# ankitkumar93/compute-war

Measured on AMD Instinct MI355X. Metric: GB/s ingested (Skein-512 + LZ4, 64 KiB blocks), higher is better.
Workload: dtype u64; 1 GPU; skein512+lz4, 1048576 x 65536 B uniform-random blocks/GPU in HBM; blocks_per_gpu=1048576, block_bytes=65536, parallelism=block-sharded x1, gather-only RCCL

## Files before the change

### compute_war_amd/csrc/lz4_kernel.hip

```cpp

#include <hip/hip_runtime.h>
#include <stdint.h>
#include <stdio.h>
#include <stdlib.h>
#include <string.h>

#include <type_traits>

#include "cw_device.h"
#include "lz_device.h"
#include "stream_scratch.h"

#ifndef HEADW_GLOBAL
#define HEADW_GLOBAL 16
#endif
#ifndef HEADW_STAGED
#define HEADW_STAGED 64
#endif

namespace cw {

using lz::Around;
using lz::around;
using lz::copy_g2g;
// ... 193 lines not shown
        const uint32_t off = c * kChunk + j * 1024 + lane * 16;
        if (c < nchunks && off < n) r.p[j] = *reinterpret_cast<const uint4 *>(g + off);
    }
}
__device__ __forceinline__ void chunk_stage(const Chunk &r, uint32_t *ring32, uint32_t c, uint32_t n, uint32_t lane)
{
#pragma unroll
    for (uint32_t j = 0; j < kPieces; j++) {
        const uint32_t off = c * kChunk + j * 1024 + lane * 16;
        if (off < n) *reinterpret_cast<uint4 *>(reinterpret_cast<uint8_t *>(ring32) + (off & (kRing - 1))) = r.p[j];
    }
}
__device__ __forceinline__ void chunk_store(const Chunk &r, uint8_t *lit, uint32_t c, uint32_t n, uint32_t lane)
{
#pragma unroll
    for (uint32_t j = 0; j < kPieces; j++) {
        const uint32_t off = c * kChunk + j * 1024 + lane * 16;
        if (off < n) {
            uint32_t *q = reinterpret_cast<uint32_t *>(lit + off);
            __builtin_nontemporal_store(r.p[j].x, q);
            __builtin_nontemporal_store(r.p[j].y, q + 1);
            __builtin_nontemporal_store(r.p[j].z, q + 2);
            __builtin_nontemporal_store(r.p[j].w, q + 3);
        }
    }
}

struct Walk {
    ScanState st;
    uint32_t knext = 0, v0 = 0;
    bool marked = false;
};

template <int NG>
__device__ __forceinline__ void probe_groups(Walk &w, const uint32_t (&pos)[kStreamGroup], const bool (&act)[kStreamGroup], uint32_t *tab,
                                             const uint32_t *ring32, uint32_t tag, uint32_t epoch)
{
    uint32_t v[NG], old[NG];
#pragma unroll
    for (int j = 0; j < NG; j++) {
        const uint32_t a0 = (pos[j] & (kRing - 1)) >> 2, a1 = (a0 + 1) & (kRing / 4 - 1);
        v[j] = __builtin_amdgcn_alignbyte(ring32[a1], ring32[a0], pos[j] & 3u);
    }
#pragma unroll
    for (int j = 0; j < NG; j++) old[j] = scan_issue(tab, tag, pos[j], v[j], act[j]);
#pragma unroll
    for (int j = 0; j < NG; j++) scan_judge(old[j], epoch, w.v0, pos[j], v[j], act[j], w.st);
}

__device__ __forceinline__ void probe_upto(Walk &w, uint32_t end, uint32_t *tab, const uint32_t *ring32, uint32_t tag, uint32_t epoch,
                                           uint32_t nprobes, const uint8_t *g, uint32_t lane)
{
    for (;;) {
        uint32_t pos[kStreamGroup], nact = 0, ngroups = 0;
        bool act[kStreamGroup];
#pragma unroll
        for (uint32_t j = 0; j < kStreamGroup; j++) {
            const uint32_t k = w.knext + 64 * j + lane;
            pos[j] = 1 + probe_delta(k);
            act[j] = k < nprobes && pos[j] < end;
            const unsigned long long m = __ballot(act[j]);
            nact += (uint32_t)__builtin_popcountll(m);
            ngroups += m != 0;
        }
        if (nact == 0) return;
        if (ngroups == 1) probe_groups<1>(w, pos, act, tab, ring32, tag, epoch);
        else if (ngroups == 2) probe_groups<2>(w, pos, act, tab, ring32, tag, epoch);
        else probe_groups<kStreamGroup>(w, pos, act, tab, ring32, tag, epoch);
        w.marked = scan_settle(g, w.st);
        w.knext += nact;
        if (w.marked || nact < 64 * kStreamGroup) return;
    }
}

__global__ void __launch_bounds__(64)
lz4_scan_stream_kernel(const uint8_t *__restrict__ src, uint32_t n, size_t src_stride, size_t nblocks,
                       uint8_t *__restrict__ dst, size_t dst_stride, uint32_t *__restrict__ sizes, uint32_t nprobes,
                       uint32_t *__restrict__ queue, uint32_t *__restrict__ counters, size_t first_block, uint32_t feed_word)
{
    __shared__ __attribute__((aligned(16))) uint32_t tab[1u << 13];
    __shared__ __attribute__((aligned(16))) uint32_t ring32[kRing / 4];
    volatile uint32_t *mailbox = ring32;
    const uint32_t lane = threadIdx.x;
    __builtin_amdgcn_s_setprio(3);
    uint32_t epoch = 15;
    const uint32_t nchunks = (n + kChunk - 1) / kChunk;
    const uint32_t hdr = 1 + (n >= 15 ? (n - 15) / 255 + 1 : 0);

    BlockFeed feed;
    const uint32_t run = n >= 65536 ? 1u : 65536u / n;
    for (size_t rel; scan_next_block(feed, rel, counters + feed_word - 2, mailbox, run, nblocks - first_block, lane);) {
        const size_t blk = first_block + rel;
        scan_begin_block(tab, epoch, lane);
        const uint8_t *g = src + blk * src_stride;
        uint8_t *out = dst + blk * dst_stride, *lit = out + hdr;
        const uint32_t tag = epoch << 28;
        Walk w;
        Chunk r0, r1, r2;

#define CW_STAGE(PREV, CUR, C)                                                                         \
        do {                                                                                           \
            const uint32_t c_ = (C);                                                                   \
            if (c_) chunk_store(PREV, lit, c_ - 1, n, lane);                                           \
            chunk_load(PREV, g, c_ + 2, nchunks, n, lane);                                             \
            chunk_stage(CUR, ring32, c_, n, lane);                                                     \
            if (c_ == 0) {                                                                             \
                w.v0 = ring32[0];                                                                      \
                if (nprobes && lane == 0) {                                                            \
                    const uint32_t h0 = w.v0 * 2654435761u;                                            \
                    atomicMax(&tab[h0 >> 19], tag | ((h0 >> 7) & 0xFFFu));             \
                }                                                                                      \
            } else {                                                                                   \
                probe_upto(w, c_ * kChunk, tab, ring32, tag, epoch, nprobes, g, lane);                 \
            }                                                                                          \
        } while (0)

        chunk_load(r0, g, 0, nchunks, n, lane);
        chunk_load(r1, g, 1, nchunks, n, lane);
        for (uint32_t c = 0; c < nchunks && !w.marked; c += 3) {
            CW_STAGE(r2, r0, c);
            if (c + 1 < nchunks && !w.marked) CW_STAGE(r0, r1, c + 1);
            if (c + 2 < nchunks && !w.marked) CW_STAGE(r1, r2, c + 2);
        }
#undef CW_STAGE
        if (!w.marked) {
            probe_upto(w, n, tab, ring32, tag, epoch, nprobes, g, lane);
            if (!w.marked) {
                const uint32_t last = (nchunks - 1) % 3;
                if (last == 0) chunk_store(r0, lit, nchunks - 1, n, lane);
                else if (last == 1) chunk_store(r1, lit, nchunks - 1, n, lane);
                else chunk_store(r2, lit, nchunks - 1, n, lane);
            }
        }
        if (w.marked) {
            scan_mark(sizes, blk, queue, counters, lane);
            continue;
        }
        if (n >= 15) {
            if (lane == 0) out[0] = 15u << 4;
            put_len(out + 1, n - 15, lane);
        } else if (lane == 0) {
            out[0] = (uint8_t)(n << 4);
        }
        if (lane == 0) sizes[blk] = hdr + n;
    }
}

__device__ __forceinline__ uint32_t probe_pos(uint32_t k)
{
    const uint32_t q = (k + 62) >> 6;
    return q * (k + 31 - 32 * q) + 1 + (uint32_t)(k != 0);
}

__device__ __forceinline__ uint32_t probe_kend(uint32_t end, uint32_t nprobes)
{
    uint32_t lo = 0, hi = nprobes;
    while (lo < hi) {
        const uint32_t mid = (lo + hi) >> 1;
        if (probe_pos(mid) < end) lo = mid + 1;
        else hi = mid;
    }
    return lo;
}

template <int NG, bool PART>
__device__ __forceinline__ bool probe_batches(uint32_t kb, uint32_t rem, uint32_t *tab, const uint32_t *ring32, uint32_t tag, uint32_t v0,
                                              const uint8_t *g, uint32_t lane)
{
    uint32_t pos[NG], v[NG], tp[NG], fp[NG], old[NG];
    unsigned long long actm[NG];
#pragma unroll
    for (int j = 0; j < NG; j++) {
        pos[j] = probe_pos(kb + 64 * j + lane);
        const uint8_t *r8 = reinterpret_cast<const uint8_t *>(ring32);
        const uint32_t lo = *reinterpret_cast<const uint32_t *>(r8 + (pos[j] & (kRing - 4)));
        const uint32_t hi = *reinterpret_cast<const uint32_t *>(r8 + ((pos[j] + 4) & (kRing - 4)));
        v[j] = __builtin_amdgcn_alignbyte(hi, lo, pos[j]);
    }
#pragma unroll
    for (int j = 0; j < NG; j++) {
        const bool act = !PART || 64 * j + lane < rem;
        actm[j] = PART ? __ballot(act) : ~0ull;
        const uint32_t h = v[j] * 2654435761u;
        fp[j] = (h >> 7) & 0xFFFu;
        tp[j] = tag | (pos[j] << 12);
        old[j] = atomicMax(&tab[act ? h >> 19 : 0u], act ? tp[j] | fp[j] : 0u);
    }
    unsigned long long hit = 0, maybe = 0;
#pragma unroll
    for (int j = 0; j < NG; j++) {
        const unsigned long long empty = __ballot(old[j] < tag);
        hit |= (__ballot(old[j] >= tp[j]) | (empty & __ballot(v[j] == v0))) & actm[j];
        const unsigned long long fm = __ballot(((old[j] ^ fp[j]) & 0xFFFu) == 0) & ~empty & actm[j];
        hit |= fm & maybe;
        maybe |= fm;
    }
    if (maybe) {
        uint32_t mcand = 0, mv = 0;
#pragma unroll
        for (int j = 0; j < NG; j++) {
            const bool f = (((PART ? actm[j] : ~0ull) >> lane) & 1u) && old[j] >= tag && ((old[j] ^ fp[j]) & 0xFFFu) == 0;
            mcand = f ? (old[j] >> 12) & 0xFFFFu : mcand;
            mv = f ? v[j] : mv;
        }
        const bool mine = (maybe >> lane) & 1u;
        hit |= __ballot(mine && ld32g(g + mcand) == mv);
    }
    return hit != 0;
}

__device__ __forceinline__ void store16_nt(uint8_t *p, uint32_t x, uint32_t y, uint32_t z, uint32_t w)
{
    typedef uint32_t u32x4 __attribute__((ext_vector_type(4)));
    u32x4 v = {x, y, z, w};
    __builtin_nontemporal_store(v, reinterpret_cast<u32x4 *>(p));
}

__device__ __forceinline__ void probe_range(Walk &w, uint32_t ke, uint32_t *tab, const uint32_t *ring32, uint32_t tag, const uint8_t *g,
                                            uint32_t lane)
{
    uint32_t kb = w.knext;
    for (; kb + 128 <= ke; kb += 128)
        if (probe_batches<2, false>(kb, 0, tab, ring32, tag, w.v0, g, lane)) { w.marked = true; return; }
    const uint32_t rem = ke - kb;
    if (rem > 64) w.marked = probe_batches<2, true>(kb, rem, tab, ring32, tag, w.v0, g, lane);
    else if (rem) w.marked = probe_batches<1, true>(kb, rem, tab, ring32, tag, w.v0, g, lane);
    w.knext = ke;
}

#ifdef CW_CLOCK_STAMP
__device__ unsigned long long g_clock_scan[4 * kClockSlots];
hipError_t lz4_clock_read(unsigned long long *out) { return hipMemcpyFromSymbol(out, HIP_SYMBOL(g_clock_scan), sizeof g_clock_scan); }
#endif

template <bool ALIGNED>
__global__ void __launch_bounds__(64)
lz4_scan_span_kernel(const uint8_t *__restrict__ src, uint32_t n, size_t src_stride, uint32_t nspans, uint8_t *__restrict__ dst,
                     size_t dst_stride, uint32_t *__restrict__ sizes, uint32_t nprobes, uint32_t *__restrict__ queue,
                     uint32_t *__restrict__ counters, uint32_t lg)
{
    CW_CLOCK_SCOPE(g_clock_scan);
    __shared__ __attribute__((aligned(16))) uint32_t tab[1u << 13];
    __shared__ __attribute__((aligned(16))) uint32_t ring32[kRing / 4];
    volatile uint32_t *mailbox = ring32;
    const uint32_t lane = threadIdx.x;
    __builtin_amdgcn_s_setprio(3);
    uint32_t epoch = 15;
    const uint32_t cmask = (1u << lg) - 1, run = 16u >> lg;
    const uint32_t hdr = 1 + (n - 15) / 255 + 1;
    const uint32_t lane16 = lane * 16;
    const uint32_t kend = probe_kend(lane * kChunk, nprobes);
    const uint32_t hdrw = (0xFFu << 16) | (((n - 15) % 255) << 24);

    for (;;) {
        __syncthreads();
        if (lane == 0) *mailbox = atomicAdd(&counters[2], 1u);
        __syncthreads();
        const uint32_t span = __builtin_amdgcn_readfirstlane(*mailbox);
        if (span >= nspans) break;
        __syncthreads();
        const size_t first = (size_t)span * run;
        const uint8_t *gs = src + first * src_stride;
        uint8_t *os = dst + first * dst_stride + (ALIGNED ? hdr - 2 : hdr);

        Walk w;
        size_t blk = first;
        uint32_t tag = 0, marks = 0;
        Chunk r0, r1, r2;
#define CW_LD(R, I)                                                                                          \
        do {                                                                                                 \
            const uint32_t i_ = (I) < 15u ? (I) : 15u;                                                       \
            const uint8_t *p_ = gs + (size_t)(i_ >> lg) * src_stride + ((i_ & cmask) << 12) + lane16;        \
            _Pragma("unroll") for (uint32_t j = 0; j < kPieces; j++) R.p[j] = *reinterpret_cast<const uint4 *>(p_ + j * 1024); \
        } while (0)
#define CW_ST(R, I)                                                                                          \
        do {                                                                                                 \
            const uint32_t i_ = (I), c_ = i_ & cmask;                                                        \
            uint8_t *p_ = os + (size_t)(i_ >> lg) * dst_stride + (c_ << 12) + lane16;                        \
            if constexpr (ALIGNED) {                                                                         \
                const uint32_t b_ = ((c_ & 1u) << 12) + lane16;  \
                uint32_t pw_[kPieces];                                                                       \
                _Pragma("unroll") for (uint32_t j = 0; j < kPieces; j++) pw_[j] = ring32[((b_ + j * 1024 - 4) & (kRing - 4)) / 4]; \
                if (c_ == 0 && lane == 0) pw_[0] = hdrw;                                                     \
                _Pragma("unroll") for (uint32_t j = 0; j < kPieces; j++) {                                   \
                    store16_nt(p_ + j * 1024, __builtin_amdgcn_alignbyte(R.p[j].x, pw_[j], 2),               \
                               __builtin_amdgcn_alignbyte(R.p[j].y, R.p[j].x, 2),                            \
                               __builtin_amdgcn_alignbyte(R.p[j].z, R.p[j].y, 2),                            \
                               __builtin_amdgcn_alignbyte(R.p[j].w, R.p[j].z, 2));                           \
                }                                                                                            \
                if (c_ == cmask && lane == 63)                                 \
                    *reinterpret_cast<uint16_t *>(p_ + (kPieces - 1) * 1024 + 16) = (uint16_t)(R.p[kPieces - 1].w >> 16); \
            } else {                                                                                         \
                _Pragma("unroll") for (uint32_t j = 0; j < kPieces; j++) {                                   \
                    uint32_t *q = reinterpret_cast<uint32_t *>(p_ + j * 1024);  \
                    __builtin_nontemporal_store(R.p[j].x, q);     __builtin_nontemporal_store(R.p[j].y, q + 1); \
                    __builtin_nontemporal_store(R.p[j].z, q + 2); __builtin_nontemporal_store(R.p[j].w, q + 3); \
                }                                                                                            \
            }                                                                                                \
        } while (0)
#define CW_FINISH()                                                                                          \
        do {                      \
            if (!w.marked) probe_range(w, nprobes, tab, ring32, tag, src + blk * src_stride, lane);          \
            if (w.marked) marks |= 1u << (uint32_t)(blk - first);         \
            else {                                                                                           \
                uint8_t *out = dst + blk * dst_stride;                                                       \
                if constexpr (ALIGNED) {                                                                     \
                    if (lane < (hdr - 2) / 16)                                                               \
                        store16_nt(out + lane16, lane ? ~0u : 0xFFFFFFF0u, ~0u, ~0u, ~0u);                   \
                } else {                                                                                     \
                    if (lane == 0) out[0] = 15u << 4;                                                        \
                    put_len(out + 1, n - 15, lane);                                                          \
                }                                                                                            \
                if (lane == 0) sizes[blk] = hdr + n;                                                         \
            }                                                                                                \
        } while (0)
#define CW_BEGIN(I)                                                                                          \
        do {                                                                                                 \
            blk = first + ((I) >> lg);                                                                       \
            scan_begin_block(tab, epoch, lane);                                                              \
            tag = epoch << 28;                                                                               \
            w = Walk();                                                                                      \
        } while (0)
#define CW_STAGE_IN(R, C)                                                                                    \
        do {                                                                                                 \
            uint8_t *p_ = reinterpret_cast<uint8_t *>(ring32) + (((C) & 1u) << 12) + lane16;                 \
            _Pragma("unroll") for (uint32_t j = 0; j < kPieces; j++) *reinterpret_cast<uint4 *>(p_ + j * 1024) = R.p[j]; \
        } while (0)
#define CW_AFTER_STAGE(C)                                                                                    \
        do {                                                                                                 \
            if ((C) == 0) {                                                                                  \
                w.v0 = ring32[0];                                                                            \
                if (nprobes && lane == 0) {                                                                  \
                    const uint32_t h0 = w.v0 * 2654435761u;                                                  \
                    atomicMax(&tab[h0 >> 19], tag | ((h0 >> 7) & 0xFFFu));                   \
                }                                                                                            \
            } else if (!w.marked) {                                                                          \
                probe_range(w, __builtin_amdgcn_readlane(kend, (C)), tab, ring32, tag, src + blk * src_stride, lane); \
            }                                                                                                \
        } while (0)
#define CW_STEP(PREV, CUR, I)                                                                                \
        do {                                                                                                 \
            const uint32_t s_ = (I), c_ = s_ & cmask;                                                        \
            CW_ST(PREV, s_ - 1);                                                                             \
            CW_LD(PREV, s_ + 2);                                                                             \
            if (c_ == 0) { CW_FINISH(); CW_BEGIN(s_); }                                                      \
            CW_STAGE_IN(CUR, c_);                                                                            \
            CW_AFTER_STAGE(c_);                                                                              \
        } while (0)

        CW_LD(r0, 0u);
        CW_LD(r1, 1u);
        CW_LD(r2, 2u);
        CW_BEGIN(0u);
        CW_STAGE_IN(r0, 0u);
        CW_AFTER_STAGE(0u);
        for (uint32_t i = 1; i < 16; i += 3) {
            CW_STEP(r0, r1, i);
            CW_STEP(r1, r2, i + 1);
            CW_STEP(r2, r0, i + 2);
        }
        CW_ST(r0, 15u);
        CW_FINISH();
        if (marks) {
            uint32_t base = 0;
            if (lane == 0) base = atomicAdd(&counters[1], (uint32_t)__builtin_popcount(marks));
            base = __builtin_amdgcn_readfirstlane(base);
            if (lane < 16 && ((marks >> lane) & 1u)) {
                sizes[first + lane] = kNeedsParse;
                queue[base + (uint32_t)__builtin_popcount(marks & ((1u << lane) - 1u))] = (uint32_t)(first + lane);
            }
        }
#undef CW_LD
#undef CW_ST
#undef CW_FINISH
#undef CW_BEGIN
#undef CW_STAGE_IN
#undef CW_AFTER_STAGE
#undef CW_STEP
    }
}

static uint32_t scan_probes(uint32_t n)
{
    if (n < kMFLimit + 1) return 0;
    const uint32_t limit = n - 11;
    uint32_t k = 0, p = 1, step = 1, nb = 64;
    while (p + step <= limit) { p += step; step = nb++ >> 6; k++; }
    return k;
}

template <bool STAGED>
__global__ void __launch_bounds__(64)
lz4_blocks_kernel(const uint8_t *__restrict__ src, uint32_t n, size_t src_stride, size_t nblocks,
                  uint8_t *__restrict__ dst, size_t dst_stride, uint32_t *__restrict__ sizes,
                  const uint32_t *__restrict__ queue, uint32_t *__restrict__ counters)
{
    extern __shared__ __attribute__((aligned(16))) uint8_t smem[];
    uint16_t *tab = reinterpret_cast<uint16_t *>(smem);
    uint8_t *lds_in = smem + kTabBytes;
    const uint32_t lane = threadIdx.x;

    const uint32_t qcount = counters[1];
    volatile uint32_t *mailbox = reinterpret_cast<volatile uint32_t *>(tab);
    for (uint32_t guard = 0; guard <= qcount; guard++) {
        __syncthreads();
        if (lane == 0) *mailbox = atomicAdd(&counters[0], 1u);
        __syncthreads();
        const uint32_t qi = __builtin_amdgcn_readfirstlane(*mailbox);
        if (qi >= qcount) break;
        const size_t blk = queue[qi];
        const uint8_t *g = src + blk * src_stride;
        uint8_t *out = dst + blk * dst_stride;

        __syncthreads();
        const uint8_t *in = STAGED ? lds_in : g;
        if (STAGED) {
            if ((reinterpret_cast<uintptr_t>(g) & 15) == 0) {
                const uint4 *g4 = reinterpret_cast<const uint4 *>(g);
                const uint32_t nvec = n >> 4;
                for (uint32_t i = lane; i < nvec; i += 64) reinterpret_cast<uint4 *>(lds_in)[i] = g4[i];
                for (uint32_t i = (nvec << 4) + lane; i < n; i += 64) lds_in[i] = g[i];
            } else {
                for (uint32_t i = lane; i < n; i += 64) lds_in[i] = g[i];
            }
        }
        for (uint32_t i = lane; i < kTabBytes / 16; i += 64) reinterpret_cast<uint4 *>(tab)[i] = make_uint4(0, 0, 0, 0);
        __syncthreads();

        uint32_t ip = 0, anchor = 0, op = 0;

        if (n >= kMFLimit + 1) {
            const uint32_t mflimit = n - kMFLimit, matchlimit = n - kLastLiterals;
            uint32_t ins = 0, s0 = 1;
            bool has_retest = false;

            for (uint32_t seq = 0; seq < n; seq++) {
                uint32_t match = 0, mpos = 0;
                bool found = false, exhausted = false;
                for (uint32_t t0 = 0;;) {
                    const uint32_t t = t0 + lane, k = t - 2;
                    const bool is_probe = t >= 2;
                    const uint32_t dk = t0 == 0 ? k : probe_delta(k), stepk = k == 0 ? 1u : (63u + k) >> 6;
                    const uint32_t pos = t == 0 ? ins : t == 1 ? ip : s0 + dk;
                    const bool dead = is_probe && s0 + dk + stepk > mflimit + 1;
                    const bool active = !dead && (is_probe || t == 0 || has_retest);
                    const uint32_t ndead = ctz64(__ballot(dead));
                    const unsigned long long amask = __ballot(active);
                    if (!amask) { exhausted = true; break; }

                    uint32_t v = 0, h = 0, old = 0;
                    if (active) {
                        v = rd32x<STAGED>(in, pos);
                        h = hash13(v);
                        old = tab[h];
                        tab[h] = (uint16_t)pos;
                    }
                    __syncthreads();
                    const bool lost = active && (tab[h] != (uint16_t)pos);
                    const uint32_t fa = ctz64(amask);
                    uint32_t m = ctz64(__ballot(lost));
                    if (m == fa) m = fa + 1;
                    const uint32_t L = m < ndead ? m : ndead;

                    const bool eq = active && t != 0 && lane < L && rd32x<STAGED>(in, old) == v;
                    const unsigned long long eqmask = __ballot(eq);
                    const uint32_t ncommit = eqmask ? ctz64(eqmask) + 1 : L;
                    if (__ballot(active && lane >= ncommit)) {
                        if (active && lane >= ncommit) tab[h] = (uint16_t)old;
                        if (active && lane < ncommit) tab[h] = (uint16_t)pos;
                    }
                    if (eqmask) {
                        const uint32_t w = ctz64(eqmask);
                        mpos = __builtin_amdgcn_readlane(pos, w);
                        match = __builtin_amdgcn_readlane(old, w);
                        found = true;
                        break;
                    }
                    if (ndead < 64 && L == ndead) { exhausted = true; break; }
                    t0 += L;
                }
                (void)exhausted;
                if (!found) break;
                ip = mpos;

                uint32_t mc, back;
                {
                    bool ok;
                    if (lane < 48) {
                        const uint32_t i = ip + kMinMatch + lane;
                        ok = i < matchlimit && in[i] == in[match + kMinMatch + lane];
                    } else {
// ... 1355 lines not shown
```

### compute_war_amd/csrc/skein_kernels.hip

```cpp

#include <hip/hip_runtime.h>
#include <stdint.h>
#include <stdlib.h>
#include <string.h>

#include "cw_device.h"
#include "stream_scratch.h"

namespace cw {

#define KS_PARITY 0x5555555555555555ULL

template <int R>
static __device__ __forceinline__ uint64_t rotl(uint64_t x)
{
    const uint32_t lo = (uint32_t)x, hi = (uint32_t)(x >> 32);
    uint32_t nlo, nhi;
    if (R == 32) { nlo = hi; nhi = lo; }
    else if (R < 32) {
        nlo = __builtin_amdgcn_alignbit(lo, hi, 32 - R);
        nhi = __builtin_amdgcn_alignbit(hi, lo, 32 - R);
    } else {
        nlo = __builtin_amdgcn_alignbit(hi, lo, 64 - R);
        nhi = __builtin_amdgcn_alignbit(lo, hi, 64 - R);
// ... 142 lines not shown
        }
        w[i] = v;
    }
}

template <int NW, bool ALIGNED16, bool RAGGED>
__global__ void __launch_bounds__(CW_SKEIN_THREADS)
skein_blocks_kernel(const uint8_t *__restrict__ src, size_t block_bytes, size_t src_stride, size_t nblocks,
                    SkeinIV iv, uint8_t *__restrict__ digests, unsigned digest_bytes)
{
    constexpr unsigned BB = NW * 8;
    const size_t gid = (size_t)blockIdx.x * blockDim.x + threadIdx.x;
    if (gid >= nblocks) return;
    const uint8_t *p = src + gid * src_stride;

    uint64_t X[NW], w[NW];
#pragma unroll
    for (int i = 0; i < NW; i++) X[i] = iv.w[i];

    const size_t nfull = block_bytes ? (block_bytes - 1) / BB : 0;
    const unsigned rem = RAGGED ? (unsigned)(block_bytes - nfull * BB) : BB;
    const size_t nsteps = nfull + 2;
    uint64_t t0 = 0, t1 = T1_FIRST | T1_MSG;

    if (!RAGGED || nfull || rem == BB) load_words<NW, ALIGNED16>(w, p);
    else load_tail<NW>(w, p, rem);

#pragma unroll 1
    for (size_t step = 0; step < nsteps; step++) {
        uint64_t nx[NW];
        if (!RAGGED) {
            const size_t nxt_step = step + 1;
            const uint64_t keep = nxt_step <= nfull ? ~0ull : 0ull;
            load_words<NW, ALIGNED16>(nx, p + (nxt_step <= nfull ? nxt_step : nfull) * BB);
#pragma unroll
            for (int k = 0; k < NW; k++) nx[k] &= keep;
        } else if (step + 1 < nfull || (step + 1 == nfull && rem == BB)) {
            load_words<NW, ALIGNED16>(nx, p + (step + 1) * BB);
        } else if (step + 1 == nfull) {
            load_tail<NW>(nx, p + (step + 1) * BB, rem);
        } else {
#pragma unroll
            for (int k = 0; k < NW; k++) nx[k] = 0;
        }
        if (step < nfull) {
            t0 += BB;
        } else if (step == nfull) {
            t0 += rem;
            t1 |= T1_FINAL;
        } else {
            t0 = 8;
            t1 = T1_FIRST | T1_FINAL | T1_OUT;
        }
        Ubi<NW>::run(X, w, t0, t1);
        t1 &= ~T1_FIRST;
#pragma unroll
        for (int k = 0; k < NW; k++) w[k] = nx[k];
    }

    uint8_t *out = digests + gid * digest_bytes;
    if (((digest_bytes | (unsigned)reinterpret_cast<uintptr_t>(out)) & 15) == 0) {
        uint4 *o4 = reinterpret_cast<uint4 *>(out);
#pragma unroll
        for (int k = 0; k < NW / 2; k++)
            if ((unsigned)(16 * k) < digest_bytes)
                o4[k] = make_uint4((uint32_t)X[2 * k], (uint32_t)(X[2 * k] >> 32), (uint32_t)X[2 * k + 1], (uint32_t)(X[2 * k + 1] >> 32));
    } else {
        for (unsigned k = 0; k < digest_bytes; k++) out[k] = (uint8_t)(X[k >> 3] >> (8 * (k & 7)));
    }
}

template <int NW, bool ALIGNED16>
__global__ void __launch_bounds__(CW_SKEIN_THREADS)
skein_lines_kernel(const uint8_t *__restrict__ src, size_t block_bytes, size_t src_stride, size_t nblocks,
                   SkeinIV iv, uint8_t *__restrict__ digests, unsigned digest_bytes)
{
    constexpr unsigned BB = NW * 8, SPL = 128 / BB, HS = SPL / 2;
    const size_t gid = (size_t)blockIdx.x * blockDim.x + threadIdx.x;
    if (gid >= nblocks) return;
    const uint8_t *p = src + gid * src_stride;

    uint64_t X[NW];
#pragma unroll
    for (int i = 0; i < NW; i++) X[i] = iv.w[i];

    const size_t nmsg = block_bytes / BB;
    const size_t total = nmsg + 1;
    uint64_t t0 = 0, t1 = T1_FIRST | T1_MSG;

    uint64_t A[HS][NW], B[HS][NW], S[HS][NW];
    auto fetch_half = [&](uint64_t (&dst)[HS][NW], size_t first) __attribute__((always_inline)) {
#pragma unroll
        for (unsigned j = 0; j < HS; j++) {
            const size_t s = first + j;
            const uint64_t keep = s < nmsg ? ~0ull : 0ull;
            load_words<NW, ALIGNED16>(dst[j], p + (s < nmsg ? s : nmsg - 1) * BB);
#pragma unroll
            for (int k = 0; k < NW; k++) dst[j][k] &= keep;
        }
    };
    auto run_half = [&](uint64_t (&buf)[HS][NW], size_t first) {
#pragma unroll
        for (unsigned j = 0; j < HS; j++) {
            const size_t s = first + j;
            if (s < total) {
                if (s + 1 < nmsg) {
                    t0 += BB;
                } else if (s + 1 == nmsg) {
                    t0 += BB;
                    t1 |= T1_FINAL;
                } else {
                    t0 = 8;
                    t1 = T1_FIRST | T1_FINAL | T1_OUT;
                }
                Ubi<NW>::run(X, buf[j], t0, t1);
                t1 &= ~T1_FIRST;
            }
        }
    };
    fetch_half(A, 0);
    fetch_half(B, HS);

#pragma unroll 1
    for (size_t first = 0; first < total; first += SPL) {
        run_half(A, first);
        fetch_half(A, first + SPL);
        fetch_half(S, first + SPL + HS);
        run_half(B, first + HS);
#pragma unroll
        for (unsigned j = 0; j < HS; j++)
#pragma unroll
            for (int k = 0; k < NW; k++) B[j][k] = S[j][k];
    }

    uint8_t *out = digests + gid * digest_bytes;
    if (((digest_bytes | (unsigned)reinterpret_cast<uintptr_t>(out)) & 15) == 0) {
        uint4 *o4 = reinterpret_cast<uint4 *>(out);
#pragma unroll
        for (int k = 0; k < NW / 2; k++)
            if ((unsigned)(16 * k) < digest_bytes)
                o4[k] = make_uint4((uint32_t)X[2 * k], (uint32_t)(X[2 * k] >> 32), (uint32_t)X[2 * k + 1], (uint32_t)(X[2 * k + 1] >> 32));
    } else {
        for (unsigned k = 0; k < digest_bytes; k++) out[k] = (uint8_t)(X[k >> 3] >> (8 * (k & 7)));
    }
}

constexpr uint32_t kSkeinSlices = 8;

#ifdef CW_CLOCK_STAMP
__device__ unsigned long long g_clock_skein[4 * kClockSlots];
hipError_t skein_clock_read(unsigned long long *out) { return hipMemcpyFromSymbol(out, HIP_SYMBOL(g_clock_skein), sizeof g_clock_skein); }
#endif

template <int NW, bool ALIGNED16>
__global__ void __launch_bounds__(CW_SKEIN_THREADS)
skein_slice_kernel(const uint8_t *__restrict__ src, size_t block_bytes, size_t src_stride, size_t nblocks, SkeinIV iv,
                   uint8_t *__restrict__ digests, unsigned digest_bytes, uint64_t *__restrict__ state, size_t s_begin, size_t s_end)
{
    CW_CLOCK_SCOPE_KEYED(g_clock_skein, s_begin / (s_end - s_begin ? s_end - s_begin : 1));
    constexpr unsigned BB = NW * 8, SPL = 128 / BB, HS = SPL / 2;
    const size_t gid = (size_t)blockIdx.x * blockDim.x + threadIdx.x;
    if (gid >= nblocks) return;
    const uint8_t *p = src + gid * src_stride;
    const size_t nmsg = block_bytes / BB, total = nmsg + 1;
    uint64_t *st = state + gid * NW;

    uint64_t X[NW];
    if (s_begin == 0) {
#pragma unroll
        for (int i = 0; i < NW; i++) X[i] = iv.w[i];
    } else {
#pragma unroll
        for (int i = 0; i < NW; i++) X[i] = st[i];
    }
    uint64_t t0 = (uint64_t)s_begin * BB, t1 = (s_begin == 0 ? T1_FIRST : 0) | T1_MSG;

    uint64_t A[HS][NW], B[HS][NW], S[HS][NW];
    auto fetch_half = [&](uint64_t (&dst)[HS][NW], size_t first) __attribute__((always_inline)) {
#pragma unroll
        for (unsigned j = 0; j < HS; j++) {
            const size_t s = first + j;
            const uint64_t keep = s < nmsg ? ~0ull : 0ull;
            load_words<NW, ALIGNED16>(dst[j], p + (s < nmsg ? s : nmsg - 1) * BB);
#pragma unroll
            for (int k = 0; k < NW; k++) dst[j][k] &= keep;
        }
    };
    auto run_half = [&](uint64_t (&buf)[HS][NW], size_t first) {
#pragma unroll
        for (unsigned j = 0; j < HS; j++) {
            const size_t s = first + j;
            if (s < s_end) {
                if (s + 1 < nmsg) {
                    t0 += BB;
                } else if (s + 1 == nmsg) {
                    t0 += BB;
                    t1 |= T1_FINAL;
                } else {
                    t0 = 8;
                    t1 = T1_FIRST | T1_FINAL | T1_OUT;
                }
                Ubi<NW>::run(X, buf[j], t0, t1);
                t1 &= ~T1_FIRST;
            }
        }
    };
    fetch_half(A, s_begin);
    fetch_half(B, s_begin + HS);
#pragma unroll 1
    for (size_t first = s_begin; first < s_end; first += SPL) {
        run_half(A, first);
        fetch_half(A, first + SPL);
        fetch_half(S, first + SPL + HS);
        run_half(B, first + HS);
#pragma unroll
        for (unsigned j = 0; j < HS; j++)
#pragma unroll
            for (int k = 0; k < NW; k++) B[j][k] = S[j][k];
    }

    if (s_end < total) {
#pragma unroll
        for (int i = 0; i < NW; i++) st[i] = X[i];
        return;
    }
    uint8_t *out = digests + gid * digest_bytes;
    if (((digest_bytes | (unsigned)reinterpret_cast<uintptr_t>(out)) & 15) == 0) {
        uint4 *o4 = reinterpret_cast<uint4 *>(out);
#pragma unroll
        for (int k = 0; k < NW / 2; k++)
            if ((unsigned)(16 * k) < digest_bytes)
                o4[k] = make_uint4((uint32_t)X[2 * k], (uint32_t)(X[2 * k] >> 32), (uint32_t)X[2 * k + 1], (uint32_t)(X[2 * k + 1] >> 32));
    } else {
        for (unsigned k = 0; k < digest_bytes; k++) out[k] = (uint8_t)(X[k >> 3] >> (8 * (k & 7)));
    }
}

namespace {
StreamScratch<DeviceBuf> slices;
}

bool skein_sliced_applies(int nw, const uint8_t *src, size_t block_bytes, size_t src_stride, size_t nblocks, const uint8_t *digests)
{
    const size_t bb = (size_t)nw * 8;
    return nblocks >= 4096 && block_bytes % bb == 0 && block_bytes / bb + 1 >= 256 &&
           ((reinterpret_cast<uintptr_t>(src) | src_stride | reinterpret_cast<uintptr_t>(digests)) & 15) == 0;
}

hipError_t skein_sliced_launch(int nw, const uint8_t *src, size_t block_bytes, size_t src_stride, size_t nblocks, const SkeinIV &iv,
                               uint8_t *digests, unsigned digest_bytes, hipStream_t stream)
{
    const size_t bb = (size_t)nw * 8, total = block_bytes / bb + 1, spl = 128 / bb;
    const Knobs kn = knobs();
    const size_t nsl = kn.skein_nslices ? (size_t)kn.skein_nslices : kSkeinSlices;
    size_t slice_steps = (total + nsl - 1) / nsl;
    slice_steps = (slice_steps + spl - 1) / spl * spl;
    auto &w = slices.at(stream);
    LaunchLock sequence(w.launch);
    const hipError_t err = w.reserve(nblocks * (size_t)nw * sizeof(uint64_t));
    if (err != hipSuccess) return err;
    uint64_t *state = w.as<uint64_t>();
    const dim3 grid((unsigned)((nblocks + CW_SKEIN_THREADS - 1) / CW_SKEIN_THREADS)), block(CW_SKEIN_THREADS);
    for (size_t b = 0; b < total; b += slice_steps) {
        const size_t e = b + slice_steps < total ? b + slice_steps : total;
        if (nw == 8)
            hipLaunchKernelGGL((skein_slice_kernel<8, true>), grid, block, 0, stream, src, block_bytes, src_stride, nblocks, iv, digests,
                               digest_bytes, state, b, e);
        else
            hipLaunchKernelGGL((skein_slice_kernel<4, true>), grid, block, 0, stream, src, block_bytes, src_stride, nblocks, iv, digests,
                               digest_bytes, state, b, e);
    }
    note_kernels(1, nw == 8 ? "cw::skein_slice_kernel<8, true>" : "cw::skein_slice_kernel<4, true>");
    return hipGetLastError();
}

template <int NW>
static __device__ __forceinline__ void load_node_words(uint64_t (&w)[NW], const uint8_t *p, size_t n)
{
#pragma unroll
    for (int i = 0; i < NW; i++) {
        uint64_t v = 0;
        if ((size_t)(8 * i + 8) <= n) __builtin_memcpy(&v, p + 8 * i, 8);
        else
            for (int b = 0; b < 8; b++)
                if ((size_t)(8 * i + b) < n) v |= (uint64_t)p[8 * i + b] << (8 * b);
        w[i] = v;
    }
}

template <int NW>
__global__ void __launch_bounds__(64)
skein_tree_kernel(const uint8_t *__restrict__ src, size_t block_bytes, size_t src_stride, size_t nblocks, SkeinIV g,
                  uint8_t *__restrict__ digests, unsigned digest_bytes, unsigned leaf, unsigned node, unsigned max_level,
                  unsigned cap_a)
{
    constexpr unsigned BB = NW * 8;
    extern __shared__ __attribute__((aligned(16))) uint8_t lvl[];
    const uint32_t lane = threadIdx.x;

    for (size_t blk = blockIdx.x; blk < nblocks; blk += gridDim.x) {
        const uint8_t *m = src + blk * src_stride;
        size_t bcnt = block_bytes;
        uint64_t S[NW];
#pragma unroll
        for (int i = 0; i < NW; i++) S[i] = 0;
        __syncthreads();
        for (unsigned height = 0;; height++) {
            if (height && bcnt == BB) {
                load_node_words<NW>(S, m, BB);
                break;
            }
            const bool last_level = height + 1 == max_level;
            const size_t node_len = last_level ? bcnt : (size_t)BB << (height ? node : leaf);
            const size_t nnodes = bcnt == 0 || last_level ? 1 : (bcnt + node_len - 1) / node_len;
            uint8_t *out = lvl + ((height & 1) ? cap_a : 0);
            for (size_t i = lane; i < nnodes; i += 64) {
                const size_t off = i * node_len, n = bcnt - off < node_len ? bcnt - off : node_len;
                uint64_t X[NW], w[NW];
#pragma unroll
                for (int k = 0; k < NW; k++) X[k] = g.w[k];
                uint64_t t0 = off, t1 = T1_FIRST | T1_MSG | ((uint64_t)(height + 1) << 48);
                for (size_t pos = 0;;) {
                    const bool fin = n - pos <= BB;
                    const size_t take = fin ? n - pos : BB;
                    load_node_words<NW>(w, m + off + pos, take);
                    t0 += take;
                    Ubi<NW>::run(X, w, t0, fin ? t1 | T1_FINAL : t1);
                    t1 &= ~T1_FIRST;
                    pos += take;
                    if (fin) break;
                }
                if (last_level) {
#pragma unroll
                    for (int k = 0; k < NW; k++) S[k] = X[k];
                } else {
#pragma unroll
                    for (int k = 0; k < NW; k++) *reinterpret_cast<uint64_t *>(out + i * BB + 8 * k) = X[k];
                }
            }
            if (last_level) break;
            __syncthreads();
            m = out;
            bcnt = nnodes * BB;
        }
        if (lane == 0) {
            uint64_t w[NW];
#pragma unroll
            for (int k = 0; k < NW; k++) w[k] = 0;
            Ubi<NW>::run(S, w, 8, T1_FIRST | T1_FINAL | T1_OUT);
            uint8_t *o = digests + blk * digest_bytes;
            for (unsigned k = 0; k < digest_bytes; k++) o[k] = (uint8_t)(S[k >> 3] >> (8 * (k & 7)));
        }
    }
}

hipError_t skein_tree_launch(int nw, const uint8_t *src, size_t block_bytes, size_t src_stride, size_t nblocks, unsigned hash_bits,
                             unsigned leaf, unsigned node, unsigned max_level, uint8_t *digests, hipStream_t stream)
{
    if (nblocks == 0) return hipSuccess;
    if ((nw != 4 && nw != 8) || leaf == 0 || node == 0 || max_level < 2 || leaf > 20 || node > 20 || max_level > 255 ||
        hash_bits == 0 || hash_bits > (unsigned)nw * 64 || hash_bits % 8)
        return hipErrorInvalidValue;
    const size_t bb = (size_t)nw * 8;
    const size_t n1 = block_bytes ? (block_bytes + (bb << leaf) - 1) / (bb << leaf) : 1;
    const size_t n2 = (n1 * bb + (bb << node) - 1) / (bb << node);
    const size_t cap_a = (n1 * bb + 15) & ~(size_t)15, cap_b = (n2 * bb + 15) & ~(size_t)15;
    if (cap_a + cap_b > 64 * 1024) return hipErrorInvalidValue;
    SkeinIV g;
    skein_compute_iv(nw, hash_bits, &g, (uint64_t)leaf | ((uint64_t)node << 8) | ((uint64_t)max_level << 16));
    const size_t grid = nblocks < 256 * 16 ? nblocks : 256 * 16;
    if (nw == 8)
        hipLaunchKernelGGL(skein_tree_kernel<8>, dim3((unsigned)grid), dim3(64), cap_a + cap_b, stream, src, block_bytes, src_stride,
                           nblocks, g, digests, hash_bits / 8, leaf, node, max_level, (unsigned)cap_a);
    else
        hipLaunchKernelGGL(skein_tree_kernel<4>, dim3((unsigned)grid), dim3(64), cap_a + cap_b, stream, src, block_bytes, src_stride,
                           nblocks, g, digests, hash_bits / 8, leaf, node, max_level, (unsigned)cap_a);
    return hipGetLastError();
}

template <int NW>
static hipError_t launch_skein(const uint8_t *src, size_t block_bytes, size_t src_stride, size_t nblocks, const SkeinIV &iv,
                               uint8_t *digests, unsigned digest_bytes, hipStream_t stream, bool lean)
{
    if (nblocks == 0) return hipSuccess;
    const dim3 grid((unsigned)((nblocks + CW_SKEIN_THREADS - 1) / CW_SKEIN_THREADS)), block(CW_SKEIN_THREADS);
    const bool aligned = ((reinterpret_cast<uintptr_t>(src) | src_stride) & 15) == 0;
    const bool ragged = block_bytes == 0 || (block_bytes % (NW * 8)) != 0;
#define CW_LAUNCH(A, R) do { hipLaunchKernelGGL((skein_blocks_kernel<NW, A, R>), grid, block, 0, stream, \
                                                src, block_bytes, src_stride, nblocks, iv, digests, digest_bytes); \
                             note_kernels(1, NW == 8 ? "cw::skein_blocks_kernel<8, " #A ", " #R ">" : "cw::skein_blocks_kernel<4, " #A ", " #R ">"); } while (0)
#define CW_LAUNCH_LINES(A) do { hipLaunchKernelGGL((skein_lines_kernel<NW, A>), grid, block, 0, stream, \
                                                   src, block_bytes, src_stride, nblocks, iv, digests, digest_bytes); \
                                note_kernels(1, NW == 8 ? "cw::skein_lines_kernel<8, " #A ">" : "cw::skein_lines_kernel<4, " #A ">"); } while (0)
    const SkeinMode mode = knobs().skein_mode;
    const bool steps = mode == SkeinMode::by_lean ? lean : mode == SkeinMode::steps;
    if (aligned && !ragged && steps) CW_LAUNCH(true, false);
    else if (aligned && !ragged) CW_LAUNCH_LINES(true);
    else if (aligned) CW_LAUNCH(true, true);
    else if (!ragged) CW_LAUNCH_LINES(false);
    else CW_LAUNCH(false, true);
#undef CW_LAUNCH
#undef CW_LAUNCH_LINES
    return hipGetLastError();
}

hipError_t skein512_launch(const uint8_t *src, size_t block_bytes, size_t src_stride, size_t nblocks, const SkeinIV &iv,
                           uint8_t *digests, unsigned digest_bytes, hipStream_t stream, bool lean)
{
    return launch_skein<8>(src, block_bytes, src_stride, nblocks, iv, digests, digest_bytes, stream, lean);
}

hipError_t skein256_launch(const uint8_t *src, size_t block_bytes, size_t src_stride, size_t nblocks, const SkeinIV &iv,
                           uint8_t *digests, unsigned digest_bytes, hipStream_t stream, bool lean)
{
    return launch_skein<4>(src, block_bytes, src_stride, nblocks, iv, digests, digest_bytes, stream, lean);
}

template <int NW>
__global__ void __launch_bounds__(CW_SKEIN_THREADS)
skein_chunks_kernel(const uint8_t *__restrict__ src, size_t src_bytes, const uint64_t *__restrict__ offsets, const uint32_t *__restrict__ perm,
                    const uint64_t *__restrict__ d_n, size_t max_chunks, SkeinIV iv, uint8_t *__restrict__ digests, unsigned digest_bytes)
{
    constexpr unsigned BB = NW * 8, NG = NW / 2 + 1;
    const size_t k = *d_n < max_chunks ? *d_n : max_chunks;
    const size_t gid = (size_t)blockIdx.x * blockDim.x + threadIdx.x;
// ... 117 lines not shown
```

Baseline: 1103 GB/s.

## Restructure LZ4 probe walk by groups and add interior Skein slice kernel

The LZ4 scan now walks probe positions in 64-lane groups, computing positions incrementally with umul24 instead of evaluating probe_pos per index. The per-lane group bound comes from a closed-form binary search, and the partial first and last groups get dedicated handling. Skein gains an INTERIOR template variant for slices that contain neither the message end nor a partial tail. That variant drops the bounds masking and finalisation branches and adds sched barriers to separate loads from compute. The cost is more template instantiations and more complex index bookkeeping, with some risk of off-by-one errors at group edges.

```diff
diff --git a/compute_war_amd/csrc/lz4_kernel.hip b/compute_war_amd/csrc/lz4_kernel.hip
--- a/compute_war_amd/csrc/lz4_kernel.hip
+++ b/compute_war_amd/csrc/lz4_kernel.hip
@@ -369,35 +369,40 @@
     return q * (k + 31 - 32 * q) + 1 + (uint32_t)(k != 0);
 }
 
-__device__ __forceinline__ uint32_t probe_kend(uint32_t end, uint32_t nprobes)
-{
-    uint32_t lo = 0, hi = nprobes;
+__device__ __forceinline__ uint32_t group_base(uint32_t q) { return q * (32 * q - 31) + 2; }
+
+__device__ __forceinline__ uint32_t group_end(uint32_t end, uint32_t qlast)
+{
+    uint32_t lo = 0, hi = qlast;
     while (lo < hi) {
         const uint32_t mid = (lo + hi) >> 1;
-        if (probe_pos(mid) < end) lo = mid + 1;
+        if (32 * mid * mid + 32 * mid + 6 <= end) lo = mid + 1;
         else hi = mid;
     }
     return lo;
 }
 
+struct SpanWalk {
+    uint32_t qnext = 0, v0 = 0;
+    bool marked = false;
+};
+
 template <int NG, bool PART>
-__device__ __forceinline__ bool probe_batches(uint32_t kb, uint32_t rem, uint32_t *tab, const uint32_t *ring32, uint32_t tag, uint32_t v0,
-                                              const uint8_t *g, uint32_t lane)
-{
-    uint32_t pos[NG], v[NG], tp[NG], fp[NG], old[NG];
-    unsigned long long actm[NG];
+__device__ __forceinline__ bool probe_batches(const uint32_t (&pos)[NG], uint32_t lo, uint32_t hi, uint32_t *tab, const uint32_t *ring32,
+                                              uint32_t tag, uint32_t v0, const uint8_t *g, uint32_t lane)
+{
+    uint32_t v[NG], tp[NG], fp[NG], old[NG];
+    const bool act = !PART || (lane >= lo && lane < hi);
+    const unsigned long long actm = PART ? __ballot(act) : ~0ull;
 #pragma unroll
     for (int j = 0; j < NG; j++) {
-        pos[j] = probe_pos(kb + 64 * j + lane);
         const uint8_t *r8 = reinterpret_cast<const uint8_t *>(ring32);
-        const uint32_t lo = *reinterpret_cast<const uint32_t *>(r8 + (pos[j] & (kRing - 4)));
-        const uint32_t hi = *reinterpret_cast<const uint32_t *>(r8 + ((pos[j] + 4) & (kRing - 4)));
-        v[j] = __builtin_amdgcn_alignbyte(hi, lo, pos[j]);
+        const uint32_t wlo = *reinterpret_cast<const uint32_t *>(r8 + (pos[j] & (kRing - 4)));
+        const uint32_t whi = *reinterpret_cast<const uint32_t *>(r8 + ((pos[j] + 4) & (kRing - 4)));
+        v[j] = __builtin_amdgcn_alignbyte(whi, wlo, pos[j]);
     }
 #pragma unroll
     for (int j = 0; j < NG; j++) {
-        const bool act = !PART || 64 * j + lane < rem;
-        actm[j] = PART ? __ballot(act) : ~0ull;
         const uint32_t h = v[j] * 2654435761u;
         fp[j] = (h >> 7) & 0xFFFu;
         tp[j] = tag | (pos[j] << 12);
@@ -407,8 +412,8 @@
 #pragma unroll
     for (int j = 0; j < NG; j++) {
         const unsigned long long empty = __ballot(old[j] < tag);
-        hit |= (__ballot(old[j] >= tp[j]) | (empty & __ballot(v[j] == v0))) & actm[j];
-        const unsigned long long fm = __ballot(((old[j] ^ fp[j]) & 0xFFFu) == 0) & ~empty & actm[j];
+        hit |= (__ballot(old[j] >= tp[j]) | (empty & __ballot(v[j] == v0))) & actm;
+        const unsigned long long fm = __ballot(((old[j] ^ fp[j]) & 0xFFFu) == 0) & ~empty & actm;
         hit |= fm & maybe;
         maybe |= fm;
     }
@@ -416,7 +421,7 @@
         uint32_t mcand = 0, mv = 0;
 #pragma unroll
         for (int j = 0; j < NG; j++) {
-            const bool f = (((PART ? actm[j] : ~0ull) >> lane) & 1u) && old[j] >= tag && ((old[j] ^ fp[j]) & 0xFFFu) == 0;
+            const bool f = act && old[j] >= tag && ((old[j] ^ fp[j]) & 0xFFFu) == 0;
             mcand = f ? (old[j] >> 12) & 0xFFFFu : mcand;
             mv = f ? v[j] : mv;
         }
@@ -433,16 +438,31 @@
     __builtin_nontemporal_store(v, reinterpret_cast<u32x4 *>(p));
 }
 
-__device__ __forceinline__ void probe_range(Walk &w, uint32_t ke, uint32_t *tab, const uint32_t *ring32, uint32_t tag, const uint8_t *g,
+__device__ __forceinline__ void probe_partial(SpanWalk &w, uint32_t q, uint32_t nprobes, uint32_t *tab, const uint32_t *ring32, uint32_t tag,
+                                              const uint8_t *g, uint32_t lane)
+{
+    asm volatile("" : "+v"(lane));
+    const uint32_t pos[1] = {q ? __umul24(q, lane) + group_base(q) : lane - 61};
+    const uint32_t left = nprobes + 62 - 64 * q;
+    w.marked = probe_batches<1, true>(pos, q ? 0u : 62u, left < 64 ? left : 64u, tab, ring32, tag, w.v0, g, lane);
+    w.qnext = q + 1;
+}
+
+__device__ __forceinline__ void probe_range(SpanWalk &w, uint32_t qe, uint32_t *tab, const uint32_t *ring32, uint32_t tag, const uint8_t *g,
                                             uint32_t lane)
 {
-    uint32_t kb = w.knext;
-    for (; kb + 128 <= ke; kb += 128)
-        if (probe_batches<2, false>(kb, 0, tab, ring32, tag, w.v0, g, lane)) { w.marked = true; return; }
-    const uint32_t rem = ke - kb;
-    if (rem > 64) w.marked = probe_batches<2, true>(kb, rem, tab, ring32, tag, w.v0, g, lane);
-    else if (rem) w.marked = probe_batches<1, true>(kb, rem, tab, ring32, tag, w.v0, g, lane);
-    w.knext = ke;
+    uint32_t q = w.qnext;
+    w.qnext = qe;
+    uint32_t p = __umul24(q, lane) + group_base(q);
+    for (; q + 2 <= qe; q += 2) {
+        const uint32_t pos[2] = {p, p + lane + (64 * q + 1)};
+        if (probe_batches<2, false>(pos, 0, 64, tab, ring32, tag, w.v0, g, lane)) { w.marked = true; return; }
+        p = pos[1] + lane + (64 * q + 65);
+    }
+    if (q < qe) {
+        const uint32_t pos[1] = {p};
+        w.marked = probe_batches<1, false>(pos, 0, 64, tab, ring32, tag, w.v0, g, lane);
+    }
 }
 
 #ifdef CW_CLOCK_STAMP
@@ -466,7 +486,8 @@
     const uint32_t cmask = (1u << lg) - 1, run = 16u >> lg;
     const uint32_t hdr = 1 + (n - 15) / 255 + 1;
     const uint32_t lane16 = lane * 16;
-    const uint32_t kend = probe_kend(lane * kChunk, nprobes);
+    const uint32_t qlast = (nprobes + 61) >> 6;
+    const uint32_t gend = group_end((lane + 1) * kChunk < n ? (lane + 1) * kChunk : n, qlast);
     const uint32_t hdrw = (0xFFu << 16) | (((n - 15) % 255) << 24);
 
     for (;;) {
@@ -480,7 +501,7 @@
         const uint8_t *gs = src + first * src_stride;
         uint8_t *os = dst + first * dst_stride + (ALIGNED ? hdr - 2 : hdr);
 
-        Walk w;
+        SpanWalk w;
         size_t blk = first;
         uint32_t tag = 0, marks = 0;
         Chunk r0, r1, r2;
@@ -516,8 +537,8 @@
             }                                                                                                \
         } while (0)
 #define CW_FINISH()                                                                                          \
-        do {                      \
-            if (!w.marked) probe_range(w, nprobes, tab, ring32, tag, src + blk * src_stride, lane);          \
+        do {  \
+            if (nprobes && !w.marked) probe_partial(w, qlast, nprobes, tab, ring32, tag, src + blk * src_stride, lane); \
             if (w.marked) marks |= 1u << (uint32_t)(blk - first);         \
             else {                                                                                           \
                 uint8_t *out = dst + blk * dst_stride;                                                       \
@@ -536,7 +557,7 @@
             blk = first + ((I) >> lg);                                                                       \
             scan_begin_block(tab, epoch, lane);                                                              \
             tag = epoch << 28;                                                                               \
-            w = Walk();                                                                                      \
+            w = SpanWalk();                                                                                  \
         } while (0)
 #define CW_STAGE_IN(R, C)                                                                                    \
         do {                                                                                                 \
@@ -551,9 +572,9 @@
                     const uint32_t h0 = w.v0 * 2654435761u;                                                  \
                     atomicMax(&tab[h0 >> 19], tag | ((h0 >> 7) & 0xFFFu));                   \
                 }                                                                                            \
-            } else if (!w.marked) {                                                                          \
-                probe_range(w, __builtin_amdgcn_readlane(kend, (C)), tab, ring32, tag, src + blk * src_stride, lane); \
+                if (qlast) probe_partial(w, 0u, nprobes, tab, ring32, tag, src + blk * src_stride, lane);    \
             }                                                                                                \
+            if (!w.marked) probe_range(w, __builtin_amdgcn_readlane(gend, (C)), tab, ring32, tag, src + blk * src_stride, lane); \
         } while (0)
 #define CW_STEP(PREV, CUR, I)                                                                                \
         do {                                                                                                 \
diff --git a/compute_war_amd/csrc/skein_kernels.hip b/compute_war_amd/csrc/skein_kernels.hip
--- a/compute_war_amd/csrc/skein_kernels.hip
+++ b/compute_war_amd/csrc/skein_kernels.hip
@@ -318,7 +318,7 @@
 hipError_t skein_clock_read(unsigned long long *out) { return hipMemcpyFromSymbol(out, HIP_SYMBOL(g_clock_skein), sizeof g_clock_skein); }
 #endif
 
-template <int NW, bool ALIGNED16>
+template <int NW, bool ALIGNED16, bool INTERIOR>
 __global__ void __launch_bounds__(CW_SKEIN_THREADS)
 skein_slice_kernel(const uint8_t *__restrict__ src, size_t block_bytes, size_t src_stride, size_t nblocks, SkeinIV iv,
                    uint8_t *__restrict__ digests, unsigned digest_bytes, uint64_t *__restrict__ state, size_t s_begin, size_t s_end)
@@ -346,17 +346,25 @@
 #pragma unroll
         for (unsigned j = 0; j < HS; j++) {
             const size_t s = first + j;
-            const uint64_t keep = s < nmsg ? ~0ull : 0ull;
-            load_words<NW, ALIGNED16>(dst[j], p + (s < nmsg ? s : nmsg - 1) * BB);
-#pragma unroll
-            for (int k = 0; k < NW; k++) dst[j][k] &= keep;
+            if constexpr (INTERIOR) {
+                load_words<NW, ALIGNED16>(dst[j], p + s * BB);
+            } else {
+                const uint64_t keep = s < nmsg ? ~0ull : 0ull;
+                load_words<NW, ALIGNED16>(dst[j], p + (s < nmsg ? s : nmsg - 1) * BB);
+#pragma unroll
+                for (int k = 0; k < NW; k++) dst[j][k] &= keep;
+            }
         }
     };
     auto run_half = [&](uint64_t (&buf)[HS][NW], size_t first) {
 #pragma unroll
         for (unsigned j = 0; j < HS; j++) {
             const size_t s = first + j;
-            if (s < s_end) {
+            if constexpr (INTERIOR) {
+                t0 += BB;
+                Ubi<NW>::run(X, buf[j], t0, t1);
+                t1 &= ~T1_FIRST;
+            } else if (s < s_end) {
                 if (s + 1 < nmsg) {
                     t0 += BB;
                 } else if (s + 1 == nmsg) {
@@ -376,8 +384,10 @@
 #pragma unroll 1
     for (size_t first = s_begin; first < s_end; first += SPL) {
         run_half(A, first);
+        if constexpr (INTERIOR) __builtin_amdgcn_sched_barrier(0);
         fetch_half(A, first + SPL);
         fetch_half(S, first + SPL + HS);
+        if constexpr (INTERIOR) __builtin_amdgcn_sched_barrier(0);
         run_half(B, first + HS);
 #pragma unroll
         for (unsigned j = 0; j < HS; j++)
@@ -385,7 +395,7 @@
             for (int k = 0; k < NW; k++) B[j][k] = S[j][k];
     }
 
-    if (s_end < total) {
+    if (INTERIOR || s_end < total) {
 #pragma unroll
         for (int i = 0; i < NW; i++) st[i] = X[i];
         return;
@@ -427,16 +437,24 @@
     if (err != hipSuccess) return err;
     uint64_t *state = w.as<uint64_t>();
     const dim3 grid((unsigned)((nblocks + CW_SKEIN_THREADS - 1) / CW_SKEIN_THREADS)), block(CW_SKEIN_THREADS);
+    bool interior_used = false;
     for (size_t b = 0; b < total; b += slice_steps) {
         const size_t e = b + slice_steps < total ? b + slice_steps : total;
-        if (nw == 8)
-            hipLaunchKernelGGL((skein_slice_kernel<8, true>), grid, block, 0, stream, src, block_bytes, src_stride, nblocks, iv, digests,
+        const bool interior = nw == 8 && (e - b) % spl == 0 && e + spl <= total - 1;
+        interior_used |= interior;
+        if (interior)
+            hipLaunchKernelGGL((skein_slice_kernel<8, true, true>), grid, block, 0, stream, src, block_bytes, src_stride, nblocks, iv, digests,
+                               digest_bytes, state, b, e);
+        else if (nw == 8)
+            hipLaunchKernelGGL((skein_slice_kernel<8, true, false>), grid, block, 0, stream, src, block_bytes, src_stride, nblocks, iv, digests,
                                digest_bytes, state, b, e);
         else
-            hipLaunchKernelGGL((skein_slice_kernel<4, true>), grid, block, 0, stream, src, block_bytes, src_stride, nblocks, iv, digests,
+            hipLaunchKernelGGL((skein_slice_kernel<4, true, false>), grid, block, 0, stream, src, block_bytes, src_stride, nblocks, iv, digests,
                                digest_bytes, state, b, e);
     }
-    note_kernels(1, nw == 8 ? "cw::skein_slice_kernel<8, true>" : "cw::skein_slice_kernel<4, true>");
+    note_kernels(1, interior_used ? "cw::skein_slice_kernel<8, true, true> + cw::skein_slice_kernel<8, true, false>"
+                    : nw == 8     ? "cw::skein_slice_kernel<8, true, false>"
+                                  : "cw::skein_slice_kernel<4, true, false>");
     return hipGetLastError();
 }
 
```

Measured after the change: 1126 GB/s (median of 6 runs). 2.1% higher.
